# landonclark97/numbotics

Measured on AMD Instinct MI355X. Metric: collision-checked configs/sec, Kinova 7-DoF + obstacles, higher is better.
Workload: dtype f64

## Files before the change

### include/nbk.h

```cpp
#ifndef NBK_H
#define NBK_H
#include <stdint.h>

#ifdef __cplusplus
extern "C" {
#endif

#define NBK_ABI_VERSION 2

enum {
    NBK_OK = 0,
    NBK_ERR_INVALID = -1,
    NBK_ERR_NO_DEVICE = -2,
    NBK_ERR_HIP = -3,
    NBK_ERR_UNSUPPORTED = -4,
    NBK_ERR_ALLOC = -5
};

enum { NBK_SPHERE = 0, NBK_CAPSULE = 1, NBK_BOX = 2, NBK_CYLINDER = 3, NBK_PLANE = 4, NBK_HULL = 5 };
enum { NBK_REVOLUTE = 0, NBK_PRISMATIC = 1 };
enum { NBK_CONNECT = 0, NBK_STEER = 1 };

#define NBK_MAX_JOINTS 32
#define NBK_MAX_DOF 32
// ... 17 lines not shown
    int32_t n_wshapes;
    const int32_t *wshape_type;
    const double *wshape_pose;
    const double *wshape_param;
    int32_t n_pairs;
    const int32_t *pair_a;
    const int32_t *pair_b;
    int32_t n_hulls;
    const int32_t *hull_vert_begin;
    const double *hull_verts;
    const int32_t *hull_face_begin;
    const double *hull_planes;
} nbk_model_desc;

typedef struct nbk_model nbk_model;

int32_t nbk_abi_version(void);
const char *nbk_status_string(int32_t status);
const char *nbk_last_error(void);
int32_t nbk_device_count(void);

int32_t nbk_model_create(const nbk_model_desc *desc, nbk_model **out);
void nbk_model_destroy(nbk_model *m);
int32_t nbk_model_num_pairs(const nbk_model *m);

int32_t nbk_model_create_movable(const nbk_model_desc *desc, double world_radius, nbk_model **out);
int32_t nbk_model_set_world_poses(nbk_model *m, const double *poses , void *stream);
int32_t nbk_model_set_world_poses_host(nbk_model *m, const double *poses );
int32_t nbk_model_world_status(const nbk_model *m, int32_t *status);
int32_t nbk_world_reach_bounds_host(const nbk_model_desc *desc, const double *poses , double *bound );

int32_t nbk_broad_kernel_used(const nbk_model *m);
int64_t nbk_broad_spec_source(const nbk_model_desc *desc, char *buf, int64_t cap);
int64_t nbk_jit_compile(const char *src, const char *arch);

int32_t nbk_fk_batch(const nbk_model *m, const double *q, int64_t B, const int32_t *path, int32_t path_len,
                     const double *local, const double *local_pose, double *T_out, void *stream);

typedef struct nbk_frameset nbk_frameset;
int32_t nbk_frameset_create(const nbk_model *m, int32_t n_frames, const int32_t *frame_joint, const double *frame_local,
                            nbk_frameset **out);
void nbk_frameset_destroy(nbk_frameset *fs);
int32_t nbk_fk_frames_batch(const nbk_model *m, const nbk_frameset *fs, const double *q, int64_t B, double *T_out,
                            void *stream);

int32_t nbk_jacobian_batch(const nbk_model *m, const double *q, int64_t B, const int32_t *path,
                           int32_t path_len, const double *local, int32_t mode, const double *pose,
                           double *J_out, void *stream);

int32_t nbk_ik_batch(const nbk_model *m, const double *pose, const double *q0, int64_t B, const int32_t *path,
                     int32_t path_len, const double *local, const double *limits, double tol, int32_t max_iter,
                     int32_t max_failures, double *q_out, uint8_t *success, double *diff_norm, int32_t *iters,
                     void *stream);

int32_t nbk_validity_batch(const nbk_model *m, const double *q, int64_t B, double threshold,
                           uint64_t *mask_bits, uint8_t *mask_bytes, void *stream);
int64_t nbk_validity_workspace_bytes(const nbk_model *m, int64_t B);
int32_t nbk_validity_batch_ws(const nbk_model *m, const double *q, int64_t B, double threshold,
                              uint64_t *mask_bits, uint8_t *mask_bytes, void *workspace,
                              int64_t workspace_bytes, void *stream);

int32_t nbk_closest_batch(const nbk_model *m, const double *q, int64_t B, double *min_dist,
                          int32_t *argmin, void *stream);

int32_t nbk_pair_distances_batch(const nbk_model *m, const double *q, int64_t B, double *dist,
                                 double *witness, void *stream);
// ... 71 lines not shown
```

### numbotics_amd/_lib.py

```python
import ctypes as C
import os

_HERE = os.path.dirname(os.path.abspath(__file__))
LIB_PATH = os.path.join(_HERE, "csrc", "libnbk.so")

NBK_OK = 0
CA_FREE, CA_COLLISION, CA_UNDECIDED, CA_DEGENERATE = 0, 1, 2, 3
STATUS = {0: "NBK_OK", -1: "NBK_ERR_INVALID", -2: "NBK_ERR_NO_DEVICE", -3: "NBK_ERR_HIP",
          -4: "NBK_ERR_UNSUPPORTED", -5: "NBK_ERR_ALLOC"}

SYMBOLS = [
    "nbk_abi_version", "nbk_status_string", "nbk_last_error", "nbk_device_count",
    "nbk_model_create", "nbk_model_destroy", "nbk_model_num_pairs",
    "nbk_fk_batch", "nbk_frameset_create", "nbk_frameset_destroy", "nbk_fk_frames_batch", "nbk_jacobian_batch", "nbk_ik_batch", "nbk_validity_batch", "nbk_validity_workspace_bytes",
    "nbk_validity_batch_ws", "nbk_closest_batch",
    "nbk_pair_distances_batch", "nbk_proximity_jacobian_batch", "nbk_pair_records_items", "nbk_edge_validity_batch",
    "nbk_edge_continuous_batch", "nbk_edge_motion_bounds_host", "nbk_selftest_math",
    "nbk_fk_batch_host", "nbk_validity_batch_host", "nbk_knn_prefix",
    "nbk_validity_scalar_host", "nbk_edge_validity_scalar_host", "nbk_spline_validity_batch",
    "nbk_spline_continuous_batch", "nbk_spline_motion_bounds_host",
    "nbk_broad_kernel_used", "nbk_broad_spec_source", "nbk_jit_compile",
    "nbk_model_create_movable", "nbk_model_set_world_poses", "nbk_model_set_world_poses_host", "nbk_model_world_status",
    "nbk_world_reach_bounds_host",
    "nbk_cloud_create", "nbk_cloud_destroy", "nbk_cloud_set_points", "nbk_cloud_status", "nbk_cloud_validity_batch",
    "nbk_cloud_clearance_batch", "nbk_cloud_cells_host",
    "nbk_edge_cloud_workspace_bytes", "nbk_edge_cloud_validity_batch",
]
MAX_SPLINE_DEGREE = 5


class ModelDesc(C.Structure):
    _fields_ = [
        ("n_q", C.c_int32), ("n_joints", C.c_int32),
        ("joint_parent", C.c_void_p), ("joint_type", C.c_void_p), ("joint_qidx", C.c_void_p),
        ("joint_rot", C.c_void_p), ("joint_trans", C.c_void_p), ("joint_slide", C.c_void_p),
        ("joint_axis", C.c_void_p), ("base_pose", C.c_void_p),
        ("n_rshapes", C.c_int32),
        ("rshape_frame", C.c_void_p), ("rshape_type", C.c_void_p), ("rshape_local", C.c_void_p),
        ("rshape_param", C.c_void_p),
        ("n_wshapes", C.c_int32),
        ("wshape_type", C.c_void_p), ("wshape_pose", C.c_void_p), ("wshape_param", C.c_void_p),
        ("n_pairs", C.c_int32),
        ("pair_a", C.c_void_p), ("pair_b", C.c_void_p),
        ("n_hulls", C.c_int32),
        ("hull_vert_begin", C.c_void_p), ("hull_verts", C.c_void_p),
        ("hull_face_begin", C.c_void_p), ("hull_planes", C.c_void_p),
    ]


class NbkError(RuntimeError):
    pass


_lib = None
# ... 106 lines not shown
```

### numbotics_amd/csrc/nbk.hip

```cpp
#include <hip/hip_runtime.h>
#include <stdint.h>
#include <math.h>
#include <stdio.h>
#include <stdlib.h>
#include <string.h>
#include <ctype.h>

#include <memory>
#include <mutex>
#include <atomic>
#include <algorithm>
#include <type_traits>
#include <vector>
#include <string>
#include <map>
#include <dlfcn.h>
#include <hip/hiprtc.h>

#include "../../include/nbk.h"
#include "nbk_device.hpp"
#include "nbk_bf32_common.hpp"
namespace nbk {
constexpr int NSUB = 256;
}
// ... 3466 lines not shown
                dir = dir.substr(0, dir.rfind('/') + 1);
                h = dlopen((dir + "libhiprtc.so").c_str(), RTLD_NOW | RTLD_LOCAL);
            }
        }
        if (h == nullptr) return;
        r.create = reinterpret_cast<decltype(r.create)>(dlsym(h, "hiprtcCreateProgram"));
        r.compile = reinterpret_cast<decltype(r.compile)>(dlsym(h, "hiprtcCompileProgram"));
        r.log_size = reinterpret_cast<decltype(r.log_size)>(dlsym(h, "hiprtcGetProgramLogSize"));
        r.log = reinterpret_cast<decltype(r.log)>(dlsym(h, "hiprtcGetProgramLog"));
        r.code_size = reinterpret_cast<decltype(r.code_size)>(dlsym(h, "hiprtcGetCodeSize"));
        r.code = reinterpret_cast<decltype(r.code)>(dlsym(h, "hiprtcGetCode"));
        r.destroy = reinterpret_cast<decltype(r.destroy)>(dlsym(h, "hiprtcDestroyProgram"));
        r.ok = r.create && r.compile && r.log_size && r.log && r.code_size && r.code && r.destroy;
    });
    return r;
}

static int32_t bf32_compile(const std::string& src, const std::string& arch, std::vector<char>& code) {
    const Rtc& r = rtc();
    if (!r.ok) { snprintf(g_err, sizeof(g_err), "hipRTC is not available"); return NBK_ERR_UNSUPPORTED; }
    static const char* const known[] = {"gfx908", "gfx90a", "gfx940", "gfx941", "gfx942", "gfx950", "gfx1030", "gfx1100", "gfx1101",
                                        "gfx1102", "gfx1200", "gfx1201"};
    bool known_arch = false;
    for (const char* k : known) known_arch = known_arch || arch == k;
    if (!known_arch) { snprintf(g_err, sizeof(g_err), "hipRTC: unsupported target '%.64s'", arch.c_str()); return NBK_ERR_UNSUPPORTED; }
    hiprtcProgram prog;
    if (r.create(&prog, src.c_str(), "k_broad_f32_spec.hip", 0, nullptr, nullptr) != HIPRTC_SUCCESS) {
        snprintf(g_err, sizeof(g_err), "hiprtcCreateProgram failed");
        return NBK_ERR_UNSUPPORTED;
    }
    const std::string arch_opt = "--offload-arch=" + arch;
    std::vector<const char*> opts = {arch_opt.c_str(), "-O3", "-std=c++17", "-ffp-contract=off"};
    const char* extra = getenv("NBK_JIT_OPTIONS");
    if (extra != nullptr && *extra) opts.push_back(extra);
    const hiprtcResult cr = r.compile(prog, (int)opts.size(), opts.data());
    if (cr != HIPRTC_SUCCESS) {
        size_t n = 0;
        std::string log;
        if (r.log_size(prog, &n) == HIPRTC_SUCCESS && n > 1) { log.resize(n); if (r.log(prog, &log[0]) != HIPRTC_SUCCESS) log.clear(); }
        snprintf(g_err, sizeof(g_err), "hipRTC compile of the specialised broadphase failed: %.200s", log.c_str());
        r.destroy(&prog);
        return NBK_ERR_UNSUPPORTED;
    }
    size_t n = 0;
    if (r.code_size(prog, &n) != HIPRTC_SUCCESS || n == 0) { r.destroy(&prog); snprintf(g_err, sizeof(g_err), "hipRTC: no code"); return NBK_ERR_UNSUPPORTED; }
    code.resize(n);
    const hiprtcResult gr = r.code(prog, code.data());
    r.destroy(&prog);
    return gr == HIPRTC_SUCCESS ? NBK_OK : NBK_ERR_UNSUPPORTED;
}

static std::string device_arch() {
    const char* ov = getenv("NBK_JIT_ARCH");
    if (ov != nullptr && *ov) return ov;
    int dev = 0;
    hipDeviceProp_t p;
    if (hipGetDevice(&dev) != hipSuccess || hipGetDeviceProperties(&p, dev) != hipSuccess) return std::string();
    std::string a(p.gcnArchName);
    return a.substr(0, a.find(':'));
}

static hipFunction_t bf32_function(const std::string& spec) {
    static std::mutex mu;
    static std::map<std::string, hipFunction_t> memo;
    int dev = 0;
    if (hipGetDevice(&dev) != hipSuccess) return nullptr;
    const std::string arch = device_arch();
// ... 103 lines not shown
        static_assert(sizeof(HullRef) == 24, "HullRef must overlay h[3]");
        memcpy(B.bytes.data() + slot, &r, sizeof(r));
    };
    for (int i = 0; i < d->n_rshapes; ++i) if (t.rs_hull[i] >= 0) patch(hs.rs_core + sizeof(double) * 6 * (size_t)i, t.rs_hull[i]);
    for (int w = 0; w < d->n_wshapes; ++w) if (t.ws_hull[w] >= 0) patch(hs.ws_core + sizeof(double) * (18 * (size_t)w + 12), t.ws_hull[w]);
}

static int32_t model_create(const nbk_model_desc* d, const double* world_radius, nbk_model** out) {
    { const int32_t rc = desc_check(d, D_ALL); if (rc != NBK_OK) return rc; }
    ModelTables t;
    { const int32_t rc = compile_tables(d, world_radius, t); if (rc != NBK_OK) return rc; }
    std::unique_ptr<nbk_model, decltype(&nbk_model_destroy)> M(new nbk_model(), nbk_model_destroy);
    Blob B;
    const HullSlots hs = pack_model(d, t, B, *M);
    hipError_t e = hipMalloc(&M->blob, B.bytes.size());
    if (e != hipSuccess) { M->blob = nullptr; hip_fail(e, "hipMalloc(model)"); return NBK_ERR_ALLOC; }
    B.resolve(M->blob);
    patch_hulls(d, t, hs, M->blob, B);
    e = hipMemcpy(M->blob, B.bytes.data(), B.bytes.size(), hipMemcpyHostToDevice);
    if (e != hipSuccess) return hip_fail(e, "hipMemcpy(model)");
    if (world_radius != nullptr) { M->movable = M->pm.movable = true; M->world_radius = *world_radius; }
    (void)hipGetDevice(&M->device);
    *out = M.release();
    return NBK_OK;
}

int32_t nbk_model_create(const nbk_model_desc* d, nbk_model** out) {
    if (d == nullptr || out == nullptr) return NBK_ERR_INVALID;
    *out = nullptr;
    if (nbk_device_count() <= 0) return NBK_ERR_NO_DEVICE;
    return model_create(d, nullptr, out);
}

int64_t nbk_broad_spec_source(const nbk_model_desc* d, char* buf, int64_t cap) {
    { const int32_t rc = desc_check(d, D_ALL); if (rc != NBK_OK) return rc; }
    ModelTables t;
    { const int32_t rc = compile_tables(d, nullptr, t); if (rc != NBK_OK) return rc; }
    if (t.spec.empty()) return 0;
    const std::string src = bf32_source(t.spec);
    if (buf != nullptr && cap > 0) {
        const size_t n = src.size() < (size_t)(cap - 1) ? src.size() : (size_t)(cap - 1);
        memcpy(buf, src.data(), n);
        buf[n] = '\0';
    }
    return (int64_t)src.size() + 1;
}

int64_t nbk_jit_compile(const char* src, const char* arch) {
    if (src == nullptr || arch == nullptr) return NBK_ERR_INVALID;
    std::vector<char> code;
    const int32_t rc = bf32_compile(src, arch, code);
    return rc == NBK_OK ? (int64_t)code.size() : rc;
}

int32_t nbk_broad_kernel_used(const nbk_model* m) { return m == nullptr ? NBK_ERR_INVALID : m->host.last_broad.load(std::memory_order_relaxed); }

void nbk_model_destroy(nbk_model* m) {
    if (m == nullptr) return;
    if (m->blob) (void)hipFree(m->blob);
    for (StreamWs* w : m->host.wss) delete w;
    if (m->host.scalar_q) (void)hipHostFree(m->host.scalar_q);
    if (m->host.scalar_out) (void)hipHostFree(m->host.scalar_out);
    if (m->host.scalar_stream) (void)hipStreamDestroy(m->host.scalar_stream);
    if (m->host.world_ev) (void)hipEventDestroy(m->host.world_ev);
    if (m->host.world_stage) (void)hipHostFree(m->host.world_stage);
    delete m;
}

extern "C" int32_t nbk_debug_narrow_profile(unsigned long long* out, int32_t reset) {
    if (out != nullptr) NBK_HIP(hipMemcpyFromSymbol(out, HIP_SYMBOL(nbk::g_narrow_prof), sizeof(unsigned long long) * 16));
    if (reset) { unsigned long long z[16] = {0}; z[13] = ~0ull; NBK_HIP(hipMemcpyToSymbol(HIP_SYMBOL(nbk::g_narrow_prof), z, sizeof(z))); }
    return NBK_OK;
}

extern "C" int32_t nbk_debug_broad_profile(unsigned long long* out, int32_t reset) {
#ifdef NBK_BF32_STAMP
    static std::vector<unsigned long long> h(16384 * 8);
    if (out != nullptr) {
// ... 1054 lines not shown
```

### numbotics_amd/csrc/nbk_bf32_common.hpp

```cpp
#ifndef NBK_BF32_COMMON_HPP
#define NBK_BF32_COMMON_HPP

#define NBK_BF32_DEV __device__ __forceinline__

namespace nbk {

constexpr int WAVE = 64;
constexpr int BQ_CAP = 512;
constexpr int CNT_STRIDE = 16;

typedef float V2f __attribute__((ext_vector_type(2)));
typedef int V2i __attribute__((ext_vector_type(2)));
struct alignas(64) Row16f { float v[16]; };

struct FTabOffsets { int rkey, rp, rcert, rptri, rneg, rnd, wkey, wtc, wp, wcert, wcin, wkey2, rho, n_reach, wlist, wbx; };
__host__ __device__ constexpr FTabOffsets ftab_offsets(int W) {
    const int w16 = W * 16;
    const int wkey = 1408, wtc = wkey + w16, rho = wtc + 5 * w16, n_reach = rho + 32, wlist = n_reach + 16;
    return FTabOffsets{0, 256, 512, 768, 896, 1152, wkey, wtc, wtc + w16, wtc + 2 * w16, wtc + 3 * w16, wtc + 4 * w16, rho, n_reach, wlist,
                       wlist + ((W + 15) & ~15)};
}

NBK_BF32_DEV V2f splat2(float x) { return V2f{x, x}; }
NBK_BF32_DEV V2f fma2(V2f a, V2f b, V2f c) { return __builtin_elementwise_fma(a, b, c); }
// ... 19 lines not shown
    const V2f s2 = splat2(s), c2 = splat2(c);
    V2f Lp[3];
#pragma unroll
    for (int r = 0; r < 3; ++r) Lp[r] = fma2(s2, V2f{jp.m2p[2 * r], jp.m2p[2 * r + 1]}, -(c2 * V2f{jp.m1p[2 * r], jp.m1p[2 * r + 1]}));
    const V2f cu = fma2(P.Rc[2], splat2(Lp[2].x), fma2(P.Rc[1], splat2(Lp[1].x), P.Rc[0] * splat2(Lp[0].x)));
    const V2f cv = fma2(P.Rc[2], splat2(Lp[2].y), fma2(P.Rc[1], splat2(Lp[1].y), P.Rc[0] * splat2(Lp[0].y)));
    const V2f ck = fma2(P.Rc[2], splat2(jp.mk[2]), fma2(P.Rc[1], splat2(jp.mk[1]), P.Rc[0] * splat2(jp.mk[0])));
    const V2f r2 = fma2(splat2(P.R2[2]), Lp[2], fma2(splat2(P.R2[1]), Lp[1], splat2(P.R2[0]) * Lp[0]));
    const float r2k = __builtin_fmaf(P.R2[2], jp.mk[2], __builtin_fmaf(P.R2[1], jp.mk[1], P.R2[0] * jp.mk[0]));
    const V2f tc = fma2(P.Rc[2], splat2(jp.toff[2]), fma2(P.Rc[1], splat2(jp.toff[1]), fma2(P.Rc[0], splat2(jp.toff[0]), P.tc)));
    const float t2 = __builtin_fmaf(P.R2[2], jp.toff[2], __builtin_fmaf(P.R2[1], jp.toff[1], __builtin_fmaf(P.R2[0], jp.toff[0], P.t2)));
    o.Rc[U] = cu; o.Rc[V] = cv; o.Rc[KZ] = ck;
    o.R2[U] = r2.x; o.R2[V] = r2.y; o.R2[KZ] = r2k;
    o.tc = tc; o.t2 = t2;
}

NBK_BF32_DEV void joint_apply_gen_p(const float* M, const float* toff, const float* sl, const XfP& P, float qk, float s, float c, XfP& o) {
    float L[9], tl[3];
#pragma unroll
    for (int e = 0; e < 9; ++e) L[e] = __builtin_fmaf(s, M[18 + e], __builtin_fmaf(-c, M[9 + e], M[e]));
#pragma unroll
    for (int i = 0; i < 3; ++i) tl[i] = __builtin_fmaf(qk, sl[i], toff[i]);
    XfP n;
#pragma unroll
    for (int j = 0; j < 3; ++j) {
        n.Rc[j] = fma2(P.Rc[2], splat2(L[6 + j]), fma2(P.Rc[1], splat2(L[3 + j]), P.Rc[0] * splat2(L[j])));
        n.R2[j] = __builtin_fmaf(P.R2[2], L[6 + j], __builtin_fmaf(P.R2[1], L[3 + j], P.R2[0] * L[j]));
    }
    n.tc = fma2(P.Rc[2], splat2(tl[2]), fma2(P.Rc[1], splat2(tl[1]), fma2(P.Rc[0], splat2(tl[0]), P.tc)));
    n.t2 = __builtin_fmaf(P.R2[2], tl[2], __builtin_fmaf(P.R2[1], tl[1], __builtin_fmaf(P.R2[0], tl[0], P.t2)));
    o = n;
}

NBK_BF32_DEV void box_slot2(V2f dx, V2f dy, V2f dz, const float* wc, const float* tb, V2i& cand, V2i& certh) {
    const V2f dd = fma2(dz, dz, fma2(dy, dy, dx * dx));
    V2f ex[3], ex2 = V2f{0.0f, 0.0f};
#pragma unroll
    for (int j = 0; j < 3; ++j) {
        const V2f pj = fma2(dz, splat2(wc[5 + 3 * j]), fma2(dy, splat2(wc[4 + 3 * j]), dx * splat2(wc[3 + 3 * j])));
        ex[j] = V2f{__builtin_fabsf(pj.x) - wc[12 + j], __builtin_fabsf(pj.y) - wc[12 + j]};
        const V2f cl = V2f{__builtin_fmaxf(ex[j].x, 0.0f), __builtin_fmaxf(ex[j].y, 0.0f)};
        ex2 = fma2(cl, cl, ex2);
    }
    const V2f mx = V2f{__builtin_fmaxf(ex[0].x, __builtin_fmaxf(ex[1].x, ex[2].x)), __builtin_fmaxf(ex[0].y, __builtin_fmaxf(ex[1].y, ex[2].y))};
    const V2i s1 = __builtin_bit_cast(V2i, dd - V2f{tb[0], tb[1]});
    const V2i s2 = __builtin_bit_cast(V2i, ex2 - V2f{tb[2], tb[3]});
    const V2i s3 = __builtin_bit_cast(V2i, ex2 - V2f{tb[4], tb[5]});
    const V2i s4 = __builtin_bit_cast(V2i, dd - V2f{tb[6], tb[7]});
    const V2i s5 = __builtin_bit_cast(V2i, mx + V2f{tb[8], tb[9]});
    const V2i nz = __builtin_bit_cast(V2i, V2f{0.0f, 0.0f} - ex2);
    const V2i mi = __builtin_bit_cast(V2i, mx);
    cand = s1 & s2;
    certh = cand & ((s3 & nz) | (mi & s5 & s4));
}

NBK_BF32_DEV void hull_slot2(V2f dx, V2f dy, V2f dz, const float* wc, const float* ob, const float* tb, V2i& cand, V2i& certh) {
    const V2f dd = fma2(dz, dz, fma2(dy, dy, dx * dx));
    V2f ex2 = V2f{0.0f, 0.0f};
#pragma unroll
    for (int j = 0; j < 3; ++j) {
        const V2f pj = fma2(dz, splat2(wc[5 + 3 * j]), fma2(dy, splat2(wc[4 + 3 * j]), dx * splat2(wc[3 + 3 * j]))) - splat2(ob[j]);
        const V2f cl = V2f{__builtin_fmaxf(__builtin_fabsf(pj.x) - ob[3 + j], 0.0f), __builtin_fmaxf(__builtin_fabsf(pj.y) - ob[3 + j], 0.0f)};
        ex2 = fma2(cl, cl, ex2);
    }
    const V2i s1 = __builtin_bit_cast(V2i, dd - V2f{tb[0], tb[1]});
    const V2i s2 = __builtin_bit_cast(V2i, ex2 - V2f{tb[2], tb[3]});
    certh = __builtin_bit_cast(V2i, dd - V2f{tb[4], tb[5]});
    cand = s1 & s2;
}

NBK_BF32_DEV void plane_slot1(float dx, float dy, float dz, const float* wc, float key2, float cert, bool& cand, bool& certh) {
    const float hc = __builtin_fmaf(dz, wc[11], __builtin_fmaf(dy, wc[10], dx * wc[9]));
// ... 162 lines not shown
```

### numbotics_amd/csrc/nbk_bf32_spec.hpp

```cpp

#define NBK_SPEC_DEV __device__ __forceinline__
#define NBK_SPEC_INLINE __attribute__((always_inline))

namespace nbk_spec {

using namespace nbk;
enum { K_BOX = 2, K_HULL = 4, K_PLANE = 5 };
enum { JK_PRISMATIC = 4 };

template <int V> struct IC { static constexpr int value = V; };
template <int B, int E, class F> NBK_SPEC_DEV void sfor(F&& f) {
    if constexpr (B < E) { f(IC<B>{}); sfor<B + 1, E>(f); }
}

template <class Spec> struct SpecRoute {
    const int* __restrict__ vp_cls;
    NBK_SPEC_DEV int cls(unsigned p) const { return vp_cls[p]; }
    NBK_SPEC_DEV int base(int c) const { return Spec::cls_base[c]; }
    NBK_SPEC_DEV int groups(int c) const { return Spec::cls_groups[c]; }
};

template <class Spec>
NBK_SPEC_DEV void broad_f32_spec(const double* __restrict__ q, long long B, const float* __restrict__ ftb, const float* __restrict__ tab,
                                 unsigned long long* __restrict__ mask_bits, unsigned char* __restrict__ mask_bytes,
                                 unsigned long long* __restrict__ q_count, unsigned long long* __restrict__ q_items, unsigned long long cap,
                                 unsigned char* ovf, const int* __restrict__ vp_cls) {
    constexpr int S = Spec::S, SB = Spec::SB, NQ = Spec::NQ, J = Spec::J, W = Spec::W;
    constexpr FTabOffsets FO = ftab_offsets(W);
    extern __shared__ double lds[];
    const int lane = threadIdx.x;
    const long long base = (long long)blockIdx.x * WAVE;
    double* lds_raw = lds;
    constexpr int qrows = NQ > (SB + 2) / 2 ? NQ : (SB + 2) / 2;
    constexpr int qcap = qrows * (WAVE * 2);
    static_assert(qcap >= BQ_CAP && qcap >= S * WAVE, "the q slab must hold the general stage's queue and one unrolled block's items");
    unsigned* lds_queue = reinterpret_cast<unsigned*>(lds_raw);
    if (base >= B) return;
    const int rows_i = (int)((B - base) < WAVE ? (B - base) : WAVE);
    stage_plain_rows(q, base, rows_i, NQ, lds_raw, lane);
    __syncthreads();
    const bool active = lane < rows_i;
    int hit = 0;
#pragma unroll
    for (int j = 0; j < NQ; ++j) hit = hit || !(__builtin_fabs(lds_raw[lane * NQ + j]) <= 1.7976931348623157e308);
    float cxa[SB], cya[SB], cza[SB];
#pragma unroll
    for (int i = 0; i < SB; ++i) { cxa[i] = 0.0f; cya[i] = 0.0f; cza[i] = 0.0f; }
    float rmax = Spec::f_reach, qabs = 0.0f;
    float qv[J];
#pragma unroll
    for (int k = 0; k < J; ++k) { qv[k] = (float)lds_raw[lane * NQ + Spec::qcol[k]]; qabs += __builtin_fabsf(qv[k]); }
    XfP T;
    {
        const float* bp = ftb + Spec::f_base;
#pragma unroll
        for (int k = 0; k < 3; ++k) { T.Rc[k] = V2f{bp[k], bp[4 + k]}; T.R2[k] = bp[8 + k]; }
        T.tc = V2f{bp[3], bp[7]}; T.t2 = bp[11];
    }
    auto shapes = [&](auto K) NBK_SPEC_INLINE {
        constexpr int k = decltype(K)::value;
        sfor<Spec::sh_begin[k], Spec::sh_begin[k + 1]>([&](auto SH) NBK_SPEC_INLINE {
            constexpr int sh = decltype(SH)::value;
            const float tl0 = ftb[Spec::f_tl + 3 * sh], tl1 = ftb[Spec::f_tl + 3 * sh + 1], tl2 = ftb[Spec::f_tl + 3 * sh + 2];
            const V2f cp = fma2(T.Rc[2], splat2(tl2), fma2(T.Rc[1], splat2(tl1), fma2(T.Rc[0], splat2(tl0), T.tc)));
            const float c2 = __builtin_fmaf(T.R2[2], tl2, __builtin_fmaf(T.R2[1], tl1, __builtin_fmaf(T.R2[0], tl0, T.t2)));
            cxa[sh] = cp.x; cya[sh] = cp.y; cza[sh] = c2;
            rmax = __builtin_fmaxf(rmax, __builtin_fmaxf(__builtin_fabsf(cp.x), __builtin_fmaxf(__builtin_fabsf(cp.y), __builtin_fabsf(c2))));
        });
    };
    shapes(IC<0>{});
    sfor<0, J>([&](auto K) NBK_SPEC_INLINE {
        constexpr int k = decltype(K)::value;
        constexpr int kind = Spec::jkind[k];
        float s = 0.0f, c = 0.0f;
        if constexpr (kind != JK_PRISMATIC) sincos_f(qv[k], s, c);
        if constexpr (kind <= 2) {
            const JPk jp = *reinterpret_cast<const JPk*>(ftb + Spec::f_pk + 20 * k);
            joint_apply_axis_p<kind>(jp, T, s, c, T);
        } else {
            joint_apply_gen_p(ftb + Spec::f_rot + 27 * k, ftb + Spec::f_trans + 3 * k, ftb + Spec::f_slide + 3 * k, T, qv[k], s, c, T);
        }
        shapes(IC<k + 1>{});
    });
    const float e2 = 2.0f * rmax * __builtin_fmaf(2.4e-7f, qabs, Spec::f_eps);
    __syncthreads();
    int qn = 0;
    const SpecRoute<Spec> route{vp_cls};
    const float* wbx_all = tab + FO.wbx;
    if (__builtin_amdgcn_ballot_w64(!(e2 <= Spec::f_e2max)) == 0ull) {
        sfor<0, Spec::NW>([&](auto WI) NBK_SPEC_INLINE {
            constexpr int wi = decltype(WI)::value;
            constexpr int w = Spec::wl[wi];
            constexpr int wk = Spec::wk[wi];
            const float* wc = ftb + Spec::f_wc + 18 * w;
            if constexpr (wk == K_BOX || wk == K_HULL) {
                const float* wb = wbx_all + w * 96;
                const float* ob = ftb + Spec::f_wobb + 6 * w;
                int cwv[SB];
                int acc_c = 0, acc_h = 0;
                sfor<0, SB / 2>([&](auto I) NBK_SPEC_INLINE {
                    constexpr int i = decltype(I)::value;
                    cwv[2 * i] = 0; cwv[2 * i + 1] = 0;
                    if constexpr (Spec::wpair(wi, 2 * i) >= 0 || Spec::wpair(wi, 2 * i + 1) >= 0) {
                        const V2f dx = V2f{cxa[2 * i], cxa[2 * i + 1]} - splat2(wc[0]);
                        const V2f dy = V2f{cya[2 * i], cya[2 * i + 1]} - splat2(wc[1]);
                        const V2f dz = V2f{cza[2 * i], cza[2 * i + 1]} - splat2(wc[2]);
                        V2i cand, certh;
                        if constexpr (wk == K_BOX) box_slot2(dx, dy, dz, wc, wb + 12 * i, cand, certh);
                        else hull_slot2(dx, dy, dz, wc, ob, wb + 12 * i, cand, certh);
                        cwv[2 * i] = cand.x; cwv[2 * i + 1] = cand.y;
                        acc_c |= cand.x | cand.y;
                        acc_h |= certh.x | certh.y;
                    }
                });
                hit = hit || (acc_h < 0);
                const bool live = active && !hit;
                if (__builtin_amdgcn_ballot_w64(acc_c < 0 && live) != 0ull) {
                    queue_room(S * WAVE, qcap, route, lds_queue, qn, base, q_count, q_items, cap, lane, ovf);
                    sfor<0, S>([&](auto A) NBK_SPEC_INLINE {
                        constexpr int a = decltype(A)::value;
                        if constexpr (Spec::wpair(wi, a) >= 0) enqueue_lanes(cwv[a] < 0 && live, (unsigned)Spec::wpair(wi, a), lds_queue, qn, lane);
                    });
                }
            } else {
                const Row16f wkey2r = *reinterpret_cast<const Row16f*>(tab + FO.wkey2 + w * 16);
                const Row16f wcertr = *reinterpret_cast<const Row16f*>(tab + FO.wcert + w * 16);
                const Row16f wkeyr = *reinterpret_cast<const Row16f*>(tab + FO.wkey + w * 16);
                const int* tab_wp = reinterpret_cast<const int*>(tab + FO.wp);
                bool c[SB];
                bool ch = false, anyc = false;
                sfor<0, S>([&](auto A) NBK_SPEC_INLINE {
                    constexpr int a = decltype(A)::value;
                    c[a] = false;
                    if constexpr (Spec::wpair(wi, a) >= 0) {
                        if constexpr (wk == K_PLANE) {
                            if (tab_wp[w * 16 + a] >= 0) plane_slot1(cxa[a] - wc[0], cya[a] - wc[1], cza[a] - wc[2], wc, wkey2r.v[a], wcertr.v[a], c[a], ch);
                        } else {
                            if (wkeyr.v[a] >= 0.0f) sphere_slot1(cxa[a] - wc[0], cya[a] - wc[1], cza[a] - wc[2], wkey2r.v[a], wcertr.v[a], c[a], ch);
                        }
                        anyc = anyc || c[a];
                    }
                });
                hit = hit || ch;
                const bool live = active && !hit;
                if (__builtin_amdgcn_ballot_w64(anyc && live) != 0ull) {
                    queue_room(S * WAVE, qcap, route, lds_queue, qn, base, q_count, q_items, cap, lane, ovf);
                    sfor<0, S>([&](auto A) NBK_SPEC_INLINE {
                        constexpr int a = decltype(A)::value;
                        if constexpr (Spec::wpair(wi, a) >= 0) enqueue_lanes(c[a] && live, (unsigned)Spec::wpair(wi, a), lds_queue, qn, lane);
                    });
                }
            }
        });
        if constexpr (Spec::rr_any) {
            sfor<0, S - 1>([&](auto A) NBK_SPEC_INLINE {
                constexpr int a = decltype(A)::value;
                if constexpr (Spec::row_slots(a) > 0) {
                    const Row16f nk = *reinterpret_cast<const Row16f*>(tab + FO.rneg + a * 16);
                    const V2f ax2 = V2f{cxa[a], cxa[a]}, ay2 = V2f{cya[a], cya[a]}, az2 = V2f{cza[a], cza[a]};
                    V2f ev[SB / 2];
                    int acc_e = 0;
                    sfor<(a + 1) / 2, SB / 2>([&](auto I) NBK_SPEC_INLINE {
                        constexpr int i = decltype(I)::value;
                        if constexpr (Spec::rr_group(a, i)) {
                            ev[i] = slot_e2(ax2 - V2f{cxa[2 * i], cxa[2 * i + 1]}, ay2 - V2f{cya[2 * i], cya[2 * i + 1]},
                                            az2 - V2f{cza[2 * i], cza[2 * i + 1]}, V2f{nk.v[2 * i], nk.v[2 * i + 1]});
                            const V2i ei = __builtin_bit_cast(V2i, ev[i]);
                            acc_e |= ei.x | ei.y;
                        }
                    });
                    if (__builtin_amdgcn_ballot_w64(acc_e < 0 && active && !hit) != 0ull) {
                        const Row16f nd = *reinterpret_cast<const Row16f*>(tab + FO.rnd + a * 16);
                        int acc_f = 0;
                        sfor<(a + 1) / 2, SB / 2>([&](auto I) NBK_SPEC_INLINE {
                            constexpr int i = decltype(I)::value;
                            if constexpr (Spec::rr_group(a, i)) {
                                const V2i fi = __builtin_bit_cast(V2i, ev[i] + V2f{nd.v[2 * i], nd.v[2 * i + 1]});
                                acc_f |= fi.x | fi.y;
                            }
                        });
                        hit = hit || (acc_f < 0);
                        const bool live = active && !hit;
                        queue_room(Spec::row_slots(a) * WAVE, qcap, route, lds_queue, qn, base, q_count, q_items, cap, lane, ovf);
                        sfor<a + 1, S>([&](auto Bb) NBK_SPEC_INLINE {
                            constexpr int b = decltype(Bb)::value;
                            if constexpr (Spec::rr_p(a, b) >= 0) {
                                const V2i ei = __builtin_bit_cast(V2i, ev[b / 2]);
                                enqueue_lanes(((b % 2) ? ei.y : ei.x) < 0 && live, (unsigned)Spec::rr_p(a, b), lds_queue, qn, lane);
                            }
                        });
                    }
                }
            });
        }
    } else {
        const bool cert_ok = e2 <= Spec::f_e2max;
        bool certh = false;
        const float* tab_wkey = tab + FO.wkey; const float* tab_wtc = tab + FO.wtc; const float* tab_wcert = tab + FO.wcert;
        const float* tab_wcin = tab + FO.wcin; const float* tab_rho = tab + FO.rho;
        const int* tab_wp = reinterpret_cast<const int*>(tab + FO.wp);
        const int* tab_rp = reinterpret_cast<const int*>(tab + FO.rp);
        const float* tab_rkey = tab + FO.rkey; const float* tab_rcert = tab + FO.rcert;
        sfor<0, Spec::NW>([&](auto WI) NBK_SPEC_INLINE {
            constexpr int wi = decltype(WI)::value;
            constexpr int w = Spec::wl[wi];
            constexpr int wk = Spec::wk[wi];
            const float* wc = ftb + Spec::f_wc + 18 * w;
            unsigned long long bits = 0ull;
            sfor<0, S>([&](auto A) NBK_SPEC_INLINE {
                constexpr int a = decltype(A)::value;
                if constexpr (Spec::wpair(wi, a) >= 0) {
                    const float dx = cxa[a] - wc[0], dy = cya[a] - wc[1], dz = cza[a] - wc[2];
                    if constexpr (wk == K_PLANE) {
                        if (tab_wp[w * 16 + a] >= 0)
                            bits |= plane_slot_gen(dx, dy, dz, wc, tab_wkey[w * 16 + a], tab_rho[a], e2, tab_wcert[w * 16 + a], certh) ? (1ull << a) : 0ull;
                    } else if constexpr (wk == K_BOX) {
                        if (tab_wkey[w * 16 + a] >= 0.0f)
// ... 46 lines not shown
```

### numbotics_amd/csrc/nbk_tables.hpp

```cpp
#pragma once

namespace nbk {

enum : unsigned {
    D_JOINTS = 1,
    D_CHAIN = 2,
    D_RSHAPES = 4,
    D_WSHAPES = 8,
    D_HULL_VERTS = 16,
    D_HULL_PLANES = 32,
    D_PAIRS = 64,
    D_MOTION = D_JOINTS | D_RSHAPES | D_HULL_VERTS | D_PAIRS,
    D_ALL = 127
};

static int32_t desc_check(const nbk_model_desc* d, unsigned parts) {
    if (d == nullptr) return NBK_ERR_INVALID;
    const int J = d->n_joints, S = d->n_rshapes, W = d->n_wshapes, P = d->n_pairs, H = d->n_hulls;
    if (d->n_q < 0 || J < 0 || S < 0 || W < 0 || P < 0 || H < 0) return NBK_ERR_INVALID;
    if (J > NBK_MAX_JOINTS || d->n_q > NBK_MAX_DOF) return NBK_ERR_UNSUPPORTED;
    if (parts & D_HULL_PLANES) parts |= D_HULL_VERTS;
    if ((parts & D_HULL_VERTS) && H > 0) {
        if (d->hull_vert_begin == nullptr || d->hull_verts == nullptr || d->hull_vert_begin[0] != 0) return NBK_ERR_INVALID;
        for (int h = 0; h < H; ++h) if (d->hull_vert_begin[h + 1] <= d->hull_vert_begin[h]) return NBK_ERR_INVALID;
// ... 451 lines not shown
        if (std::sqrt(n2) > freach) freach = std::sqrt(n2);
    }
    if (world_radius != nullptr && *world_radius > freach) freach = *world_radius;
    t.f_wobb = (int)ftab.size();
    for (int w = 0; w < W; ++w)
        for (int e = 0; e < 6; ++e) {
            const double v = t.ws_hull[w] >= 0 ? t.hull_obb[6 * (size_t)t.ws_hull[w] + e] : 0.0;
            ftab.push_back(e < 3 ? (float)v : (float)v * (1.0f + 2.4e-7f));
        }
    while (ftab.size() % 4 != 0) ftab.push_back(0.0f);
    t.f_pk = (int)ftab.size();
    ftab.resize(ftab.size() + 20 * (size_t)(J > 8 ? J : 8), 0.0f);
    for (int k = 0; k < J; ++k) {
        float* fp = &ftab[t.f_pk + 20 * (size_t)k];
        pack_joint_rot(d->joint_rot + 27 * (size_t)k, t.joint_kind[k], fp);
        for (int e = 0; e < 3; ++e) fp[16 + e] = (float)d->joint_trans[3 * k + e];
    }
    t.f_meta = (int)ftab.size();
    for (int k = 0; k < 8; ++k) {
        const unsigned v = k < J ? ((unsigned)t.joint_kind[k] | ((unsigned)d->joint_qidx[k] << 8)) : 0u;
        float fv; memcpy(&fv, &v, 4);
        ftab.push_back(fv);
    }
    t.f_chain = (J >= 1 && J <= 8 && S <= 16) ? 1 : 0;
    for (int k = 0; k < J && t.f_chain; ++k) if (t.load[k] != (k == 0 ? -1 : -2) || t.save[k] != -1) t.f_chain = 0;
    const double rel = 50.0 * (J + 2) * 16.0 * 5.96e-8;
    t.f_eps = (float)(rel > 1e-4 ? rel : 1e-4);
    t.f_reach = (float)(freach > 1e-3 ? freach : 1e-3);
    t.f_e2max = 2.0f * t.f_reach * (t.f_eps + 2.4e-7f * 64.0f) * (1.0f + 1e-6f);
}

constexpr int SPEC_MAX_WORLD = 2;

static std::string bf32_spec_text(const nbk_model_desc* d, const ModelTables& t) {
    const int S = d->n_rshapes, J = d->n_joints, W = d->n_wshapes, P = d->n_pairs;
    if (!t.f_chain || P == 0 || S < 1 || S > 16 || J < 1 || J > 8) return std::string();
    std::vector<int> rrp((size_t)S * S, -1), wlist;
    std::vector<int> wslot_of(W > 0 ? W : 1, -1);
    for (int j = 0; j < P; ++j) {
        const int* bt = &t.bq_tab[4 * j];
        if (bt[3] != 1 && wslot_of[bt[1]] < 0) { wslot_of[bt[1]] = 0; wlist.push_back(bt[1]); }
    }
    std::sort(wlist.begin(), wlist.end());
    if ((int)wlist.size() > SPEC_MAX_WORLD) return std::string();
    const int NW = (int)wlist.size();
    for (int i = 0; i < NW; ++i) wslot_of[wlist[i]] = i;
    std::vector<int> wp((size_t)(NW > 0 ? NW : 1) * S, -1);
    bool rr_any = false;
    for (int j = 0; j < P; ++j) {
        const int* bt = &t.bq_tab[4 * j];
        const int a = bt[0] / 3;
        if (bt[3] == 1) {
            const int b = bt[1] / 3, lo = a < b ? a : b, hi = a < b ? b : a;
            rrp[(size_t)lo * S + hi] = bt[2];
            rr_any = true;
        } else {
            wp[(size_t)wslot_of[bt[1]] * S + a] = bt[2];
        }
    }
    std::string o;
    char buf[512];
    auto add = [&](const char* fmt, auto... v) { snprintf(buf, sizeof(buf), fmt, v...); o += buf; };
    auto arr = [&](const char* name, const std::vector<int>& v) {
        add("    static constexpr int %s[] = {", name);
        for (size_t i = 0; i < v.size(); ++i) add(i ? ", %d" : "%d", v[i]);
        if (v.empty()) o += "-1";
        o += "};\n";
    };
    const int SB = S <= 8 ? 8 : (S <= 12 ? 12 : 16);
    o += "struct Spec {\n";
    add("    static constexpr int S = %d, SB = %d, NQ = %d, J = %d, W = %d, NW = %d;\n", S, SB, d->n_q, J, W, NW);
    arr("jkind", std::vector<int>(t.joint_kind.begin(), t.joint_kind.begin() + J));
    arr("qcol", std::vector<int>(d->joint_qidx, d->joint_qidx + J));
    arr("sh_begin", t.begin);
    add("    static constexpr int f_rot = 0, f_pk = %d, f_tl = %d, f_base = %d, f_wc = %d, f_wobb = %d, f_trans = %d, f_slide = %d;\n",
        t.f_pk, t.f_tl, t.f_base, t.f_wc, t.f_wobb, t.f_trans, t.f_slide);
    add("    static constexpr float f_eps = %af, f_reach = %af, f_e2max = %af;\n", (double)t.f_eps, (double)t.f_reach, (double)t.f_e2max);
    add("    static constexpr bool rr_any = %s;\n", rr_any ? "true" : "false");
    arr("rrp_", rrp);
    std::vector<int> wk;
    for (int w : wlist) wk.push_back(t.ws_kind[w]);
    arr("wl", wlist);
    arr("wk", wk);
    arr("wp_", wp);
    arr("cls_base", std::vector<int>(t.cls_base, t.cls_base + 4));
    std::vector<int> groups(t.cls_groups, t.cls_groups + 4);
    for (int& g : groups) g = g > 0 ? g : 1;
    arr("cls_groups", groups);
    o += "    static constexpr int rr_p(int a, int b) { return a >= 0 && b < S && a < b ? rrp_[a * S + b] : -1; }\n"
         "    static constexpr int wpair(int wi, int a) { return a < S ? wp_[wi * S + a] : -1; }\n"
         "    static constexpr bool rr_group(int a, int i) { return rr_p(a, 2 * i) >= 0 || rr_p(a, 2 * i + 1) >= 0; }\n"
         "    static constexpr int row_slots(int a) { int n = 0; for (int b = a + 1; b < S; ++b) n += rr_p(a, b) >= 0 ? 1 : 0; return n; }\n"
         "};\n";
    return o;
}

static void hull_tables(const nbk_model_desc* d, ModelTables& t) {
    const int S = d->n_rshapes, W = d->n_wshapes, H = d->n_hulls;
    auto inscribed = [&](int kind, const double* cc, int hull) {
        double r = 0.0;
        if (kind == K_BOX) r = std::min(cc[0], std::min(cc[1], cc[2]));
        else if (kind == K_CYL) r = std::min(cc[3], cc[0]);
        else if (kind == K_HULL) {
            const int f0 = d->hull_face_begin[hull], f1 = d->hull_face_begin[hull + 1];
            r = f1 > f0 ? INFINITY : 0.0;
            for (int f = f0; f < f1; ++f) r = std::min(r, d->hull_planes[4 * (size_t)f + 3]);
            r *= (1.0 - 1e-9);
        } else if (kind == K_PLANE) return 0.0;
        if (!(r > 0.0)) r = 0.0;
        return r + cc[4];
    };
    t.rs_in.assign(S > 0 ? S : 1, 0.0); t.ws_in.assign(W > 0 ? W : 1, 0.0);
    for (int i = 0; i < S; ++i) t.rs_in[i] = inscribed(t.rs_kind[i], &t.rs_core[6 * (size_t)i], t.rs_hull[i]);
    for (int w = 0; w < W; ++w) t.ws_in[w] = inscribed(t.ws_kind[w], &t.ws_core[18 * (size_t)w + 12], t.ws_hull[w]);
    t.hull_off.assign(H > 0 ? H : 1, 0);
    for (int h = 0; h < H; ++h) {
        const double* v = d->hull_verts + 3 * (size_t)d->hull_vert_begin[h];
        const int n = d->hull_vert_begin[h + 1] - d->hull_vert_begin[h];
        t.hull_blob.insert(t.hull_blob.end(), &t.hull_obb[6 * h], &t.hull_obb[6 * h] + 6);
        t.hull_off[h] = t.hull_blob.size();
        t.hull_blob.insert(t.hull_blob.end(), v, v + 3 * (size_t)n);
    }
}

static int32_t compile_tables(const nbk_model_desc* d, const double* world_radius, ModelTables& t) {
    compile_geometry(d, t);
    { const int32_t rc = check_limits(d, t); if (rc != NBK_OK) return rc; }
    { const int32_t rc = joint_tables(d, t); if (rc != NBK_OK) return rc; }
    queue_groups(d, t);
    float_tables(d, world_radius, t);
    t.spec = bf32_spec_text(d, t);
    hull_tables(d, t);
    return NBK_OK;
}

}
```

### numbotics_amd/engine.py

```python
import ctypes as C

import numpy as np

from . import _lib
from ._lib import NbkError


def _torch():
    import torch
    return torch


def _require_gpu():
    torch = _torch()
    if not torch.cuda.is_available():
        raise NbkError("no GPU visible: the numbotics_amd device path has no CPU fallback")
    return torch


class _Staged:

    def __init__(self, x, n_cols, what="q"):
        torch = _require_gpu()
        self.numpy = not torch.is_tensor(x)
# ... 78 lines not shown
        raise ValueError(f"control points must have shape (S, n, {n_q}), got {c.shape}")
    S, n = c.shape[:2]
    k = int(degree)
    if not 1 <= k < n:
        raise ValueError("degree must be at least 1 and less than the number of control points")
    kn = _host_f64(knots, n + k + 1)
    d, keep = model_desc(model)
    mu = np.zeros((S, n - k, int(d.n_pairs)), dtype=np.float64)
    _lib.check(_lib.load().nbk_spline_motion_bounds_host(C.byref(d), c.ctypes.data, S, n, k, kn.ctypes.data, mu.ctypes.data),
               "nbk_spline_motion_bounds_host")
    del keep
    return mu


def _world_poses_host(poses, n_wshapes):
    a = np.asarray(poses, dtype=np.float64)
    if a.ndim == 3 and a.shape[1:] == (4, 4):
        a = a[:, :3, :]
    if a.shape not in ((n_wshapes, 12), (n_wshapes, 3, 4)):
        raise ValueError(f"world poses must have shape ({n_wshapes}, 12) or ({n_wshapes}, 3, 4), got {a.shape}")
    return np.ascontiguousarray(a).reshape(n_wshapes, 12)


def world_reach_bounds(model, poses=None):
    W = model.n_wshapes
    ps = _world_poses_host(model.wshape_pose if poses is None else poses, W)
    d, keep = model_desc(model)
    out = np.full((int(d.n_pairs),), -np.inf, dtype=np.float64)
    _lib.check(_lib.load().nbk_world_reach_bounds_host(C.byref(d), ps.ctypes.data, out.ctypes.data), "nbk_world_reach_bounds_host")
    del keep
    return out


class DeviceModel:

    def __init__(self, model, movable=False, world_radius=None):
        kin = getattr(model, "kin", model)
        scene = model if hasattr(model, "kin") else None
        if world_radius is not None and not movable:
            raise ValueError("world_radius is meaningful for movable=True only")
        if movable:
            if scene is None:
                raise ValueError("a movable descriptor needs a SceneModel")
            if world_radius is None:
                from numbotics_amd.robots.model import default_world_radius
                world_radius = default_world_radius(scene)
            world_radius = float(world_radius)
            if not (0.0 <= world_radius < np.inf):
                raise ValueError(f"world_radius must be finite and >= 0, got {world_radius}")
        _require_gpu()
        lib = _lib.load()
        self.kin, self.scene = kin, scene
        self.movable, self.world_radius = bool(movable), world_radius
        d, keep = model_desc(model)
        h = C.c_void_p()
        if movable:
            _lib.check(lib.nbk_model_create_movable(C.byref(d), world_radius, C.byref(h)), "nbk_model_create_movable")
        else:
            _lib.check(lib.nbk_model_create(C.byref(d), C.byref(h)), "nbk_model_create")
        del keep
        self._h = h
        self._lib = lib
        self.n_q = kin.n_q
        self.n_pairs = scene.n_pairs if scene is not None else 0

    def set_world_poses(self, poses, stream_ordered=False):
# ... 434 lines not shown
```

Before: 9.308 billion.

## Specialize axis-aligned world boxes and keep joint values in registers in spec kernel

Adds a compile-time flag per static world box marking it identity-rotated, so the box test skips the rotation projection and uses the raw offsets. Joint configurations for small DOF counts (at most 8) are loaded straight into registers instead of being staged through LDS, which removes two block barriers. Also adds diagnostic macros to disable stages, a movable-spec source export, and splitting of the JIT options string into separate flags. The aligned check relies on exact float equality, and the register path issues uncoalesced per-lane row loads.

```diff
diff --git a/include/nbk.h b/include/nbk.h
--- a/include/nbk.h
+++ b/include/nbk.h
@@ -73,6 +73,7 @@
 
 int32_t nbk_broad_kernel_used(const nbk_model *m);
 int64_t nbk_broad_spec_source(const nbk_model_desc *desc, char *buf, int64_t cap);
+int64_t nbk_broad_spec_source_movable(const nbk_model_desc *desc, double world_radius, char *buf, int64_t cap);
 int64_t nbk_jit_compile(const char *src, const char *arch);
 
 int32_t nbk_fk_batch(const nbk_model *m, const double *q, int64_t B, const int32_t *path, int32_t path_len,
diff --git a/numbotics_amd/_lib.py b/numbotics_amd/_lib.py
--- a/numbotics_amd/_lib.py
+++ b/numbotics_amd/_lib.py
@@ -19,7 +19,7 @@
     "nbk_fk_batch_host", "nbk_validity_batch_host", "nbk_knn_prefix",
     "nbk_validity_scalar_host", "nbk_edge_validity_scalar_host", "nbk_spline_validity_batch",
     "nbk_spline_continuous_batch", "nbk_spline_motion_bounds_host",
-    "nbk_broad_kernel_used", "nbk_broad_spec_source", "nbk_jit_compile",
+    "nbk_broad_kernel_used", "nbk_broad_spec_source", "nbk_broad_spec_source_movable", "nbk_jit_compile",
     "nbk_model_create_movable", "nbk_model_set_world_poses", "nbk_model_set_world_poses_host", "nbk_model_world_status",
     "nbk_world_reach_bounds_host",
     "nbk_cloud_create", "nbk_cloud_destroy", "nbk_cloud_set_points", "nbk_cloud_status", "nbk_cloud_validity_batch",
diff --git a/numbotics_amd/csrc/nbk.hip b/numbotics_amd/csrc/nbk.hip
--- a/numbotics_amd/csrc/nbk.hip
+++ b/numbotics_amd/csrc/nbk.hip
@@ -3522,7 +3522,15 @@
     const std::string arch_opt = "--offload-arch=" + arch;
     std::vector<const char*> opts = {arch_opt.c_str(), "-O3", "-std=c++17", "-ffp-contract=off"};
     const char* extra = getenv("NBK_JIT_OPTIONS");
-    if (extra != nullptr && *extra) opts.push_back(extra);
+    std::vector<std::string> extras;
+    if (extra != nullptr) {
+        std::string cur;
+        for (const char* c = extra; ; ++c) {
+            if (*c == ' ' || *c == '\0') { if (!cur.empty()) extras.push_back(cur); cur.clear(); if (*c == '\0') break; }
+            else cur.push_back(*c);
+        }
+    }
+    for (const std::string& e : extras) opts.push_back(e.c_str());
     const hiprtcResult cr = r.compile(prog, (int)opts.size(), opts.data());
     if (cr != HIPRTC_SUCCESS) {
         size_t n = 0;
@@ -3692,10 +3700,10 @@
     return model_create(d, nullptr, out);
 }
 
-int64_t nbk_broad_spec_source(const nbk_model_desc* d, char* buf, int64_t cap) {
+static int64_t spec_source(const nbk_model_desc* d, const double* world_radius, char* buf, int64_t cap) {
     { const int32_t rc = desc_check(d, D_ALL); if (rc != NBK_OK) return rc; }
     ModelTables t;
-    { const int32_t rc = compile_tables(d, nullptr, t); if (rc != NBK_OK) return rc; }
+    { const int32_t rc = compile_tables(d, world_radius, t); if (rc != NBK_OK) return rc; }
     if (t.spec.empty()) return 0;
     const std::string src = bf32_source(t.spec);
     if (buf != nullptr && cap > 0) {
@@ -3704,6 +3712,11 @@
         buf[n] = '\0';
     }
     return (int64_t)src.size() + 1;
+}
+int64_t nbk_broad_spec_source(const nbk_model_desc* d, char* buf, int64_t cap) { return spec_source(d, nullptr, buf, cap); }
+int64_t nbk_broad_spec_source_movable(const nbk_model_desc* d, double world_radius, char* buf, int64_t cap) {
+    if (!(world_radius >= 0.0 && world_radius <= 1.7976931348623157e308)) return NBK_ERR_INVALID;
+    return spec_source(d, &world_radius, buf, cap);
 }
 
 int64_t nbk_jit_compile(const char* src, const char* arch) {
diff --git a/numbotics_amd/csrc/nbk_bf32_common.hpp b/numbotics_amd/csrc/nbk_bf32_common.hpp
--- a/numbotics_amd/csrc/nbk_bf32_common.hpp
+++ b/numbotics_amd/csrc/nbk_bf32_common.hpp
@@ -75,12 +75,15 @@
     o = n;
 }
 
+template <bool ALIGNED = false>
 NBK_BF32_DEV void box_slot2(V2f dx, V2f dy, V2f dz, const float* wc, const float* tb, V2i& cand, V2i& certh) {
     const V2f dd = fma2(dz, dz, fma2(dy, dy, dx * dx));
     V2f ex[3], ex2 = V2f{0.0f, 0.0f};
 #pragma unroll
     for (int j = 0; j < 3; ++j) {
-        const V2f pj = fma2(dz, splat2(wc[5 + 3 * j]), fma2(dy, splat2(wc[4 + 3 * j]), dx * splat2(wc[3 + 3 * j])));
+        V2f pj;
+        if constexpr (ALIGNED) pj = j == 0 ? dx : (j == 1 ? dy : dz);
+        else pj = fma2(dz, splat2(wc[5 + 3 * j]), fma2(dy, splat2(wc[4 + 3 * j]), dx * splat2(wc[3 + 3 * j])));
         ex[j] = V2f{__builtin_fabsf(pj.x) - wc[12 + j], __builtin_fabsf(pj.y) - wc[12 + j]};
         const V2f cl = V2f{__builtin_fmaxf(ex[j].x, 0.0f), __builtin_fmaxf(ex[j].y, 0.0f)};
         ex2 = fma2(cl, cl, ex2);
diff --git a/numbotics_amd/csrc/nbk_bf32_spec.hpp b/numbotics_amd/csrc/nbk_bf32_spec.hpp
--- a/numbotics_amd/csrc/nbk_bf32_spec.hpp
+++ b/numbotics_amd/csrc/nbk_bf32_spec.hpp
@@ -1,3 +1,29 @@
+
+#ifdef NBK_SPEC_NO_ALIGNED
+#define NBK_SPEC_ALIGNED 0
+#else
+#define NBK_SPEC_ALIGNED 1
+#endif
+#ifdef NBK_SPEC_NO_QREG
+#define NBK_SPEC_QREG 0
+#else
+#define NBK_SPEC_QREG 1
+#endif
+#ifdef NBK_SPEC_DIAG_NO_WORLD
+#define NBK_SPEC_WORLD 0
+#else
+#define NBK_SPEC_WORLD 1
+#endif
+#ifdef NBK_SPEC_DIAG_NO_RR
+#define NBK_SPEC_RR 0
+#else
+#define NBK_SPEC_RR 1
+#endif
+#ifdef NBK_SPEC_DIAG_NO_ENQUEUE
+#define NBK_SPEC_ENQUEUE 0
+#else
+#define NBK_SPEC_ENQUEUE 1
+#endif
 
 #define NBK_SPEC_DEV __device__ __forceinline__
 #define NBK_SPEC_INLINE __attribute__((always_inline))
@@ -37,19 +63,28 @@
     unsigned* lds_queue = reinterpret_cast<unsigned*>(lds_raw);
     if (base >= B) return;
     const int rows_i = (int)((B - base) < WAVE ? (B - base) : WAVE);
-    stage_plain_rows(q, base, rows_i, NQ, lds_raw, lane);
-    __syncthreads();
     const bool active = lane < rows_i;
+    constexpr bool QREG = NBK_SPEC_QREG != 0 && NQ <= 8;
+    double qd[QREG ? NQ : 1];
+    if constexpr (QREG) {
+        const double* row = q + (base + (active ? lane : 0)) * NQ;
+#pragma unroll
+        for (int j = 0; j < NQ; ++j) qd[j] = row[j];
+    } else {
+        stage_plain_rows(q, base, rows_i, NQ, lds_raw, lane);
+        __syncthreads();
+    }
+    auto qat = [&](int j) NBK_SPEC_INLINE { if constexpr (QREG) return qd[j]; else return lds_raw[lane * NQ + j]; };
     int hit = 0;
 #pragma unroll
-    for (int j = 0; j < NQ; ++j) hit = hit || !(__builtin_fabs(lds_raw[lane * NQ + j]) <= 1.7976931348623157e308);
+    for (int j = 0; j < NQ; ++j) hit = hit || !(__builtin_fabs(qat(j)) <= 1.7976931348623157e308);
     float cxa[SB], cya[SB], cza[SB];
 #pragma unroll
     for (int i = 0; i < SB; ++i) { cxa[i] = 0.0f; cya[i] = 0.0f; cza[i] = 0.0f; }
     float rmax = Spec::f_reach, qabs = 0.0f;
     float qv[J];
 #pragma unroll
-    for (int k = 0; k < J; ++k) { qv[k] = (float)lds_raw[lane * NQ + Spec::qcol[k]]; qabs += __builtin_fabsf(qv[k]); }
+    for (int k = 0; k < J; ++k) { qv[k] = (float)qat(Spec::qcol[k]); qabs += __builtin_fabsf(qv[k]); }
     XfP T;
     {
         const float* bp = ftb + Spec::f_base;
@@ -83,12 +118,12 @@
         shapes(IC<k + 1>{});
     });
     const float e2 = 2.0f * rmax * __builtin_fmaf(2.4e-7f, qabs, Spec::f_eps);
-    __syncthreads();
+    if constexpr (!QREG) __syncthreads();
     int qn = 0;
     const SpecRoute<Spec> route{vp_cls};
     const float* wbx_all = tab + FO.wbx;
     if (__builtin_amdgcn_ballot_w64(!(e2 <= Spec::f_e2max)) == 0ull) {
-        sfor<0, Spec::NW>([&](auto WI) NBK_SPEC_INLINE {
+        sfor<0, NBK_SPEC_WORLD ? Spec::NW : 0>([&](auto WI) NBK_SPEC_INLINE {
             constexpr int wi = decltype(WI)::value;
             constexpr int w = Spec::wl[wi];
             constexpr int wk = Spec::wk[wi];
@@ -106,7 +141,7 @@
                         const V2f dy = V2f{cya[2 * i], cya[2 * i + 1]} - splat2(wc[1]);
                         const V2f dz = V2f{cza[2 * i], cza[2 * i + 1]} - splat2(wc[2]);
                         V2i cand, certh;
-                        if constexpr (wk == K_BOX) box_slot2(dx, dy, dz, wc, wb + 12 * i, cand, certh);
+                        if constexpr (wk == K_BOX) box_slot2<NBK_SPEC_ALIGNED != 0 && Spec::wbox_aligned[wi] != 0>(dx, dy, dz, wc, wb + 12 * i, cand, certh);
                         else hull_slot2(dx, dy, dz, wc, ob, wb + 12 * i, cand, certh);
                         cwv[2 * i] = cand.x; cwv[2 * i + 1] = cand.y;
                         acc_c |= cand.x | cand.y;
@@ -115,7 +150,7 @@
                 });
                 hit = hit || (acc_h < 0);
                 const bool live = active && !hit;
-                if (__builtin_amdgcn_ballot_w64(acc_c < 0 && live) != 0ull) {
+                if (NBK_SPEC_ENQUEUE && __builtin_amdgcn_ballot_w64(acc_c < 0 && live) != 0ull) {
                     queue_room(S * WAVE, qcap, route, lds_queue, qn, base, q_count, q_items, cap, lane, ovf);
                     sfor<0, S>([&](auto A) NBK_SPEC_INLINE {
                         constexpr int a = decltype(A)::value;
@@ -143,7 +178,7 @@
                 });
                 hit = hit || ch;
                 const bool live = active && !hit;
-                if (__builtin_amdgcn_ballot_w64(anyc && live) != 0ull) {
+                if (NBK_SPEC_ENQUEUE && __builtin_amdgcn_ballot_w64(anyc && live) != 0ull) {
                     queue_room(S * WAVE, qcap, route, lds_queue, qn, base, q_count, q_items, cap, lane, ovf);
                     sfor<0, S>([&](auto A) NBK_SPEC_INLINE {
                         constexpr int a = decltype(A)::value;
@@ -152,7 +187,7 @@
                 }
             }
         });
-        if constexpr (Spec::rr_any) {
+        if constexpr (Spec::rr_any && NBK_SPEC_RR != 0) {
             sfor<0, S - 1>([&](auto A) NBK_SPEC_INLINE {
                 constexpr int a = decltype(A)::value;
                 if constexpr (Spec::row_slots(a) > 0) {
@@ -181,8 +216,8 @@
                         });
                         hit = hit || (acc_f < 0);
                         const bool live = active && !hit;
-                        queue_room(Spec::row_slots(a) * WAVE, qcap, route, lds_queue, qn, base, q_count, q_items, cap, lane, ovf);
-                        sfor<a + 1, S>([&](auto Bb) NBK_SPEC_INLINE {
+                        if (NBK_SPEC_ENQUEUE) queue_room(Spec::row_slots(a) * WAVE, qcap, route, lds_queue, qn, base, q_count, q_items, cap, lane, ovf);
+                        sfor<NBK_SPEC_ENQUEUE ? a + 1 : S, S>([&](auto Bb) NBK_SPEC_INLINE {
                             constexpr int b = decltype(Bb)::value;
                             if constexpr (Spec::rr_p(a, b) >= 0) {
                                 const V2i ei = __builtin_bit_cast(V2i, ev[b / 2]);
diff --git a/numbotics_amd/csrc/nbk_tables.hpp b/numbotics_amd/csrc/nbk_tables.hpp
--- a/numbotics_amd/csrc/nbk_tables.hpp
+++ b/numbotics_amd/csrc/nbk_tables.hpp
@@ -507,7 +507,7 @@
 
 constexpr int SPEC_MAX_WORLD = 2;
 
-static std::string bf32_spec_text(const nbk_model_desc* d, const ModelTables& t) {
+static std::string bf32_spec_text(const nbk_model_desc* d, const ModelTables& t, bool movable) {
     const int S = d->n_rshapes, J = d->n_joints, W = d->n_wshapes, P = d->n_pairs;
     if (!t.f_chain || P == 0 || S < 1 || S > 16 || J < 1 || J > 8) return std::string();
     std::vector<int> rrp((size_t)S * S, -1), wlist;
@@ -558,6 +558,13 @@
     arr("wl", wlist);
     arr("wk", wk);
     arr("wp_", wp);
+    std::vector<int> aligned;
+    for (int w : wlist) {
+        bool id = !movable && t.ws_kind[w] == K_BOX;
+        for (int e = 0; e < 9 && id; ++e) id = t.ftab[t.f_wc + 18 * (size_t)w + 3 + e] == (e % 4 == 0 ? 1.0f : 0.0f);
+        aligned.push_back(id ? 1 : 0);
+    }
+    arr("wbox_aligned", aligned);
     arr("cls_base", std::vector<int>(t.cls_base, t.cls_base + 4));
     std::vector<int> groups(t.cls_groups, t.cls_groups + 4);
     for (int& g : groups) g = g > 0 ? g : 1;
@@ -604,7 +611,7 @@
     { const int32_t rc = joint_tables(d, t); if (rc != NBK_OK) return rc; }
     queue_groups(d, t);
     float_tables(d, world_radius, t);
-    t.spec = bf32_spec_text(d, t);
+    t.spec = bf32_spec_text(d, t, world_radius != nullptr);
     hull_tables(d, t);
     return NBK_OK;
 }
diff --git a/numbotics_amd/engine.py b/numbotics_amd/engine.py
--- a/numbotics_amd/engine.py
+++ b/numbotics_amd/engine.py
@@ -134,6 +134,29 @@
     return out
 
 
+def broad_spec_source(model, movable=False, world_radius=None):
+    lib = _lib.load()
+    d, keep = model_desc(model)
+    if movable:
+        if world_radius is None:
+            from numbotics_amd.robots.model import default_world_radius
+            world_radius = default_world_radius(model)
+        fn = lib.nbk_broad_spec_source_movable
+        fn.argtypes, fn.restype = [C.c_void_p, C.c_double, C.c_char_p, C.c_int64], C.c_int64
+        call = lambda buf, cap: fn(C.byref(d), float(world_radius), buf, cap)
+    else:
+        call = lambda buf, cap: lib.nbk_broad_spec_source(C.byref(d), buf, cap)
+    n = call(None, 0)
+    if n < 0:
+        _lib.check(int(n), "nbk_broad_spec_source")
+    if n == 0:
+        return None
+    buf = C.create_string_buffer(int(n))
+    call(buf, n)
+    del keep
+    return buf.value
+
+
 class DeviceModel:
 
     def __init__(self, model, movable=False, world_radius=None):
```

Measured after the change: 10.11 billion, median of 6. +8.6%, better.
